# MaxLayar/Ray-Tracing-Extended

Hardware: AMD Instinct MI355X
Metric: Mrays/s (higher is better)
Workload: dtype f32; 1 GPU; configs[2]: Chess pieces x17 (100,440 triangles, BVH4), 1920x1080, 64 rays/pixel/frame (1024 spp = 16 frames), 8 bounces, PCG, FLAT_CHUNKS semantics; decomposition=single GPU, rays_per_frame=243378252, triangles=100440, chunks=7448, spheres=0

## Files before the change

ray-tracing-extended_amd/csrc/rt_api.hip:

```cpp
#include <hip/hip_runtime.h>

#include <algorithm>
#include <chrono>
#include <cfloat>
#include <cmath>
#include <condition_variable>
#include <deque>
#include <mutex>
#include <cstdarg>
#include <cstdio>
#include <cstring>
#include <ctime>
#include <string>
#include <thread>
#include <vector>

#include "rt_kernels.hpp"
#include "rt_stream.hpp"
namespace rtk {
const void* stream_kernel(bool counting, bool philox, bool compact, bool triangles);
const void* cam_stream_kernel(bool philox, bool compact, bool triangles);
}
#include "rt_geom.hpp"
#include "rt_bvh_gpu.hpp"
// ... 579 lines not shown
        return b ? lvl3(std::true_type{}) : lvl3(std::false_type{});
    };
    return a ? lvl2(std::true_type{}) : lvl2(std::false_type{});
}

struct LaunchPlan {
    rtk::DeviceScene S{}; rtk::FrameArgs F{}; rtk::StreamArgs A{};
    const void* fn = nullptr; size_t lds = 0;
    int grid = 1, batch = 1, ntiles = 0, sample_lanes_log2 = 0;
    bool philox = false, stream = false, tile_kernel = false, stream_sync = false, cam_table = false, record_costs = false;
};

int fill_scene(rt_ctx* c, rtk::DeviceScene& S)
{
    S.sph_geom = c->d_sph_geom.p; S.sph_mat = c->d_sph_mat.p; S.nodes = c->d_nodes.p; S.nodes_h = c->d_nodes_h.p;
    S.tri_geo = c->d_tri_geo.p; S.tri_nrm = c->d_tri_nrm.p; S.chunk_mat = c->d_chunk_mat.p; S.chunk_box = c->d_chunk_box.p;
    S.raw_tris = c->d_raw_tris.p; S.raw_chunk_range = c->d_raw_range.p;
    S.ns = (int)c->n_spheres; S.nn = (int)c->n_nodes;
    if (c->n_nodes >= ((size_t)1 << 25) || c->n_tris >= ((size_t)1 << 32) / 48)
        return fail(c, -7, "scene too large for 32-bit record offsets (%zu BVH nodes)", c->n_nodes);
    S.nt = (int)c->n_tris;
    S.nm = (int)c->n_chunks;
    return 0;
}

int tile_stack_cap(const rt_ctx* c)
{
    int cap = std::max(1, c->bvh.maxStack);
    if (c->opt_lds_stack > 0) cap = std::min(cap, c->opt_lds_stack);
    return std::min(cap, 64);
}

int plan_launch(rt_ctx* c, Variant var, int kernel, const rt_params* cams, int n_frames, LaunchPlan& P)
{
    rtk::DeviceScene& S = P.S; rtk::FrameArgs& F = P.F; rtk::StreamArgs& A = P.A;
    { int r = fill_scene(c, S); if (r) return r; }

    F.p = c->params;
    F.row0 = c->target_row0; F.nrows = c->target_rows; F.row_stride = c->target_row_stride;
    F.tile_w_log2 = 3;
    F.tiles_x = (c->target_w + 7) / 8; F.tiles_y = (c->target_rows + 7) / 8;
    if (kernel == 0 && c->opt_tile_w_log2 != 3) {
        F.tile_w_log2 = c->opt_tile_w_log2;
        const int tw = 1 << F.tile_w_log2, th = 64 >> F.tile_w_log2;
        F.tiles_x = (c->target_w + tw - 1) / tw; F.tiles_y = (c->target_rows + th - 1) / th;
    }
    const bool philox = P.philox = c->params.rngMode == RT_RNG_PHILOX && c->params.numRaysPerPixel >= 1;
    if (philox && var == Variant::Flat) return fail(c, -2, "the flat validation kernel implements the PCG stream only");
    if (philox) kernel = 1;
    if (philox && (c->target_w > 65535 || c->target_rows > 65535)) return fail(c, -7, "the Philox mode addresses at most 65535 x 65535 pixels per context");
    if (philox && (c->params.numRaysPerPixel > 65000 || c->params.maxBounceCount > 32000))
        return fail(c, -7, "the Philox mode takes at most 65000 rays per pixel per frame and 32000 bounces (sample and bounce share one signed 32-bit register)");
    const bool stream = P.stream = kernel == 1 && var != Variant::Flat && c->params.numRaysPerPixel >= 1
                                   && c->target_w <= 65535 && c->target_rows <= 65535;
    const bool tile_kernel = P.tile_kernel = !stream && var != Variant::Flat;
    F.stack_cap = tile_kernel ? tile_stack_cap(c)
                              : std::max(1, c->bvh.maxStack) + (stream ? 3 : 0);
    const bool six_waves = stream && !philox && var == Variant::Fast && c->opt_compact_nodes != 0 && c->n_nodes > 0;
    const int stream_stack = c->opt_stream_stack > 0 ? c->opt_stream_stack : (six_waves ? 24 : 30);
    const bool stream_spill = stream && F.stack_cap > stream_stack;
    if (stream_spill) F.stack_cap = stream_stack;
    F.full_sort = c->opt_full_sort;
    bool fixed_origin = camera_origin_is_fixed(c->params);
    if (cams) for (int f = 0; f < n_frames; ++f) fixed_origin = fixed_origin && camera_origin_is_fixed(cams[f]);
    F.fixed_origin = fixed_origin ? 1 : 0;
    F.out_frame = c->d_frame.p; F.accum = c->d_accum.p;
    F.tile_counter = c->d_tile_counter; F.counters = c->d_counters;

    const size_t lds = P.lds = var == Variant::Flat ? 0
                                       : (size_t)F.stack_cap * 64 * sizeof(uint32_t) * rtk::kWavesPerBlock
                                         + (stream ? (size_t)rtk::kGroupMax * sizeof(uint2) * rtk::kWavesPerBlock : 0);
    if (lds > 160 * 1024) return fail(c, -7, "BVH needs a %d-entry traversal stack: exceeds the 160 KiB LDS", F.stack_cap);
    const bool counting = var == Variant::Counting;
    const bool compact = c->opt_compact_nodes != 0;
    P.cam_table = cams != nullptr;
    const void* fn = P.fn = var == Variant::Flat ? (const void*)rtk::k_trace<false, true>
                   : stream ? (cams ? rtk::cam_stream_kernel(philox, compact, c->n_nodes > 0)
                                    : rtk::stream_kernel(counting, philox, compact, c->n_nodes > 0))
                   : c->n_nodes == 0
                            ? dispatch3(counting, false, false, [](auto C, auto, auto) { return (const void*)rtk::k_trace<decltype(C)::value, false, false, 6>; })
                            : dispatch3(counting, false, compact, [](auto C, auto, auto H) { return (const void*)rtk::k_trace<decltype(C)::value, false, decltype(H)::value>; });
    if (lds > 64 * 1024) RT_HIP(c, hipFuncSetAttribute(fn, hipFuncAttributeMaxDynamicSharedMemorySize, (int)lds));
    int per_cu = 0;
    RT_HIP(c, hipOccupancyMaxActiveBlocksPerMultiprocessor(&per_cu, fn, rtk::kBlock, lds));
    if (per_cu < 1) return fail(c, -7, "kernel does not fit a CU (LDS %zu B)", lds);
    P.ntiles = F.tiles_x * F.tiles_y;
    P.sample_lanes_log2 = !philox ? 0 : c->params.numRaysPerPixel >= 16 ? 4 : c->params.numRaysPerPixel >= 4 ? 2 : 0;
    const bool stream_sync = P.stream_sync = stream && (c->opt_tile_sync || philox);
    if (cams && !stream_sync) return fail(c, -7, "per-frame cameras: no k_cam_stream launch for this target");
    const size_t frames_in_queue = ((stream_sync && c->opt_frame_batch != 1) ? (size_t)std::max(1, std::min(n_frames, 64)) : 1) << P.sample_lanes_log2;
    const int want = (int)std::min<size_t>(((size_t)P.ntiles * frames_in_queue + rtk::kWavesPerBlock - 1) / rtk::kWavesPerBlock, (size_t)1 << 20);
    if (c->opt_blocks_per_cu > 0) per_cu = std::min(per_cu, c->opt_blocks_per_cu);
    const int grid = P.grid = std::max(1, std::min(want, per_cu * c->n_cu));
    A.shade_threshold = std::max(1, std::min(64, c->opt_shade_threshold));
    A.total_pixels = (unsigned int)P.ntiles * 64u;
    A.tile_sync = stream_sync ? 1 : 0;
    A.sample_lanes_log2 = P.sample_lanes_log2;
    A.tiles_per_fetch = std::max(1, std::min(rtk::kGroupMax, c->opt_tiles_per_fetch));
    A.guide_div = 1;
    A.node_min = std::max(1, std::min(64, c->opt_node_min));
    const unsigned int gstack_stride = (unsigned int)grid * rtk::kBlock;
    if (philox) {
        RT_HIP(c, c->d_park.ensure((size_t)grid * rtk::kWavesPerBlock * (size_t)A.tiles_per_fetch * 192));
        F.park = c->d_park.p;
    }
    if (stream_spill) {
        RT_HIP(c, c->d_gstack.ensure((size_t)(c->bvh.maxStack + 3 - F.stack_cap) * gstack_stride));
        F.gstack = c->d_gstack.p; F.gstack_stride = gstack_stride;
    }
    if (tile_kernel && c->bvh.maxStack > F.stack_cap) {
        RT_HIP(c, c->d_gstack.ensure((size_t)(c->bvh.maxStack - F.stack_cap) * gstack_stride));
        F.gstack = c->d_gstack.p; F.gstack_stride = gstack_stride;
// ... 1328 lines not shown
```

ray-tracing-extended_amd/csrc/rt_kernels.hpp:

```cpp
#pragma once
#include <cstddef>
#include <type_traits>
#include "rt_math.hpp"
#include "bvh.hpp"
#include "../../include/rt.h"

namespace rtk {

using rtm::v3;

struct DeviceScene {
    const float4* sph_geom;
    const float4* sph_mat;
    const float4* nodes;
    const float4* nodes_h;
    const float4* tri_geo;
    const float4* tri_nrm;
    const float4* chunk_mat;
    const float4* chunk_box;
    const float*  raw_tris;
    const uint32_t* raw_chunk_range;
    int ns, nn, nt, nm;
};

// ... 16 lines not shown
    float4* out_frame;
    float4* accum;
    float* park;
    const uint4* primary;
    const float4* focus;
    unsigned int* tile_counter;
    unsigned long long* counters;
};

constexpr uint32_t kNone = 0xFFFFFFFFu;
constexpr uint32_t kTriBit = 0x80000000u;

struct Hit {
    float    t;
    uint32_t id;
    float    u, v;
};

struct TravStack {
    uint32_t* lds; uint32_t* glb; int cap; unsigned int stride;
    __device__ __forceinline__ void push(int& sp, uint32_t v) const
    {
        if (sp < cap) lds[sp * 64] = v; else glb[(size_t)(sp - cap) * stride] = v;
        ++sp;
    }
    __device__ __forceinline__ uint32_t pop(int& sp) const
    {
        --sp;
        return sp < cap ? lds[sp * 64] : glb[(size_t)(sp - cap) * stride];
    }
};

__device__ __forceinline__ unsigned long long ballot_(bool pred) { return __builtin_amdgcn_ballot_w64(pred); }
__device__ __forceinline__ unsigned long long ballot2_(bool a, bool b) { return __builtin_amdgcn_ballot_w64(a) & __builtin_amdgcn_ballot_w64(b); }

#define RT_REGION_LIST(X) X(loop) X(fetch) X(shade) X(hit) X(hit_sphere) X(hit_checker) X(hit_scatter) X(env) X(env_sun) X(camera) X(pixel_done) \
                          X(take) X(refill) X(setup) X(setup_list) X(burst) X(burstiter) X(nodeloop) X(node) X(node_spill) X(node_pop) X(leaf) X(tri) \
                          X(tri_accept) X(tri_tie) X(tri_chunk) X(prologue) X(verify) X(epilogue) X(camera_dof) X(camera_focus) X(setup_spheres)
enum Region : int {
#define RT_X(NAME) R_##NAME,
    RT_REGION_LIST(RT_X)
#undef RT_X
    kRegionsUsed
};
constexpr int kNumRegions = 32;
static_assert(kRegionsUsed <= kNumRegions, "rt_stats.regionExecs holds 32 regions");
struct Counters { uint32_t rays, sph, nodes, tris, hits; uint32_t phase_lanes[5], phase_execs[5]; uint32_t region[kNumRegions]; };
constexpr int kNumCounters = 15 + kNumRegions;

#ifdef RT_MARKERS
#define RT_MARK(TEXT) asm volatile("; RTMARK " TEXT)
#define RT_RARE_PATH() asm volatile("; RTRARE")
#define RT_RARE_PATH_EXPR() ({ asm volatile("; RTRARE"); 0; })
#else
#define RT_MARK(TEXT) do { } while (0)
#define RT_RARE_PATH() do { } while (0)
#define RT_RARE_PATH_EXPR() 0
#endif
#define RT_REGION_BEGIN(NAME) do { RT_MARK("begin " #NAME); if (COUNT) { const unsigned long long rm_ = rtk::ballot_(true); \
                                   if ((unsigned)__builtin_ctzll(rm_) == (threadIdx.x & 63u)) cnt.region[rtk::R_##NAME]++; } } while (0)
#define RT_REGION_END(NAME) RT_MARK("end " #NAME)

template <bool COUNT>
__device__ __forceinline__ void phase_tick(Counters& cnt, int k)
{
    if (COUNT) {
        cnt.phase_lanes[k]++;
        const unsigned long long m = ballot_(1);
        if ((unsigned)(__builtin_ctzll(m)) == (threadIdx.x & 63u)) cnt.phase_execs[k]++;
    }
}

__device__ __forceinline__ v3 ld3(const float* p) { return rtm::mk(p[0], p[1], p[2]); }

__device__ __forceinline__ bool ray_bounding_box(v3 o, v3 inv, v3 bmin, v3 bmax)
{
    float tminx = (bmin.x - o.x) * inv.x, tminy = (bmin.y - o.y) * inv.y, tminz = (bmin.z - o.z) * inv.z;
    float tmaxx = (bmax.x - o.x) * inv.x, tmaxy = (bmax.y - o.y) * inv.y, tmaxz = (bmax.z - o.z) * inv.z;
    float t1x = rtm::fmin_(tminx, tmaxx), t1y = rtm::fmin_(tminy, tmaxy), t1z = rtm::fmin_(tminz, tmaxz);
    float t2x = rtm::fmax_(tminx, tmaxx), t2y = rtm::fmax_(tminy, tmaxy), t2z = rtm::fmax_(tminz, tmaxz);
    float tNear = rtm::fmax_(rtm::fmax_(t1x, t1y), t1z);
    float tFar  = rtm::fmin_(rtm::fmin_(t2x, t2y), t2z);
    return tNear <= tFar;
}

struct SphereA { float a, den, rden; bool den_ok; };
__device__ __forceinline__ SphereA sphere_a(float a)
{
    SphereA s; s.a = a; s.den = 2.0f * a;
    s.den_ok = s.den >= 0x1p-60f && s.den <= 0x1p60f;
    s.rden = rtm::rcp_mid(s.den);
    return s;
}
__device__ __forceinline__ bool ray_sphere(v3 o, v3 d, const SphereA& sa, v3 centre, float radius, float& dst)
{
    v3 oc = o - centre;
    float b = 2.0f * rtm::dot(oc, d);
    float c = rtm::dot(oc, oc) - radius * radius;
    float disc = b * b - 4.0f * sa.a * c;
    if (disc >= 0.0f) {
        const float num = -b - rtm::sqrt_(disc);
        const float an = __builtin_fabsf(num);
        const float q0 = num * sa.rden;
        float q = __builtin_fmaf(__builtin_fmaf(-q0, sa.den, num), sa.rden, q0);
        q = (num == 0.0f) ? q0 : q;
        if (!(sa.den_ok && (num == 0.0f || (an >= 0x1p-60f && an <= 0x1p60f)))) { RT_COLD_PATH(); q = num / sa.den; }
        dst = q;
        return dst >= 0.0f;
    }
    return false;
}

__device__ __forceinline__ bool ray_triangle(v3 o, v3 d, v3 A, v3 eAB, v3 eAC, v3 n, float& dst, float& u, float& v)
{
    v3 ao = o - A;
    v3 dao = rtm::cross(ao, d);
    float det = -rtm::dot(d, n);
    float inv = rtm::rcp_mid(det);
    if (det > 0x1p100f) { RT_COLD_PATH(); inv = 1.0f / det; }
    dst = rtm::dot(ao, n) * inv;
    u = rtm::dot(eAC, dao) * inv;
    v = -rtm::dot(eAB, dao) * inv;
    float w = 1.0f - u - v;
    return det >= 1e-6f && dst >= 0.0f && u >= 0.0f && v >= 0.0f && w >= 0.0f;
}


template <bool H> struct RaySlabT;
template <> struct RaySlabT<false> {
    v3 inv;
    v3 oinv;
    uint32_t nx, ny, nz;
    uint32_t fx, fy, fz;
};
template <> struct RaySlabT<true> {
    v3 inv, oinv;
    uint32_t nxy, fxy, zo;
};
using RaySlab = RaySlabT<false>;

template <bool H = false>
__device__ __forceinline__ RaySlabT<H> make_slab(v3 o, v3 d)
{
    RaySlabT<H> r;
    r.inv = rtm::mk(rtm::rcp_(d.x), rtm::rcp_(d.y), rtm::rcp_(d.z));
    r.oinv = rtm::mk(o.x * r.inv.x, o.y * r.inv.y, o.z * r.inv.z);
    if constexpr (H) {
        r.nxy = (d.x < 0.0f ? 16u : 0u) + (d.y < 0.0f ? 32u : 0u);
        r.fxy = 48u - r.nxy;
        r.zo = d.z < 0.0f ? 80u : 64u;
    } else {
        r.nx = d.x < 0.0f ? 48u : 0u;
        r.ny = d.y < 0.0f ? 64u : 16u;
        r.nz = d.z < 0.0f ? 80u : 32u;
        r.fx = 48u - r.nx; r.fy = 80u - r.ny; r.fz = 112u - r.nz;
    }
    return r;
}

typedef _Float16 rt_half2 __attribute__((ext_vector_type(2)));
__device__ __forceinline__ rt_half2 as_half2(uint32_t u) { return __builtin_bit_cast(rt_half2, u); }

template <bool H>
__device__ __forceinline__ void node_step(const float4* __restrict__ nodes, uint32_t cur, const RaySlabT<H>& r, float best_t, bool full_sort,
                                          float& t0, float& t1, float& t2, float& t3,
                                          uint32_t& c0, uint32_t& c1, uint32_t& c2, uint32_t& c3)
{
    const char* nb = reinterpret_cast<const char*>(nodes);
    const uint32_t base = cur << 7;
    const float INF = __builtin_inff();
    if constexpr (H) {
        const uint4 na = *reinterpret_cast<const uint4*>(nb + (base + r.nxy)), fa = *reinterpret_cast<const uint4*>(nb + (base + r.fxy));
        const uint4 zz = *reinterpret_cast<const uint4*>(nb + (base + r.zo));
        const uint4 ch = *reinterpret_cast<const uint4*>(nb + (base + 96u));
        const float4 og = *reinterpret_cast<const float4*>(nb + (base + 112u));
        c0 = ch.x; c1 = ch.y; c2 = ch.z; c3 = ch.w;
#ifdef RT_PROBE_LOADS
        for (int k_ = 0; k_ < RT_PROBE_LOADS; ++k_) (void)*reinterpret_cast<const volatile uint32_t*>(nb + (base + 124u));
#endif
#ifdef RT_PROBE_VALU
        { float pa_ = r.inv.x; for (int k_ = 0; k_ < RT_PROBE_VALU; ++k_) asm volatile("v_fma_f32 %0, %0, %0, %0" : "+v"(pa_)); }
#endif
#ifdef RT_PROBE_VALU_HALF
        { float pa_ = r.inv.x; for (int k_ = 0; k_ < RT_PROBE_VALU_HALF; ++k_) asm volatile("v_max_f32 %0, %0, %0" : "+v"(pa_)); }
#endif
        const float kx = __builtin_fmaf(og.x, r.inv.x, -r.oinv.x), ky = __builtin_fmaf(og.y, r.inv.y, -r.oinv.y), kz = __builtin_fmaf(og.z, r.inv.z, -r.oinv.z);
#define RT_SLABH(XW, YW, ZNW, ZFW, E, TK)                                                                                 \
        {                                                                                                                \
            const float nx_ = __builtin_fmaf((float)as_half2(na.XW).E, r.inv.x, kx), fx_ = __builtin_fmaf((float)as_half2(fa.XW).E, r.inv.x, kx); \
            const float ny_ = __builtin_fmaf((float)as_half2(na.YW).E, r.inv.y, ky), fy_ = __builtin_fmaf((float)as_half2(fa.YW).E, r.inv.y, ky); \
            const float nz_ = __builtin_fmaf((float)as_half2(zz.ZNW).E, r.inv.z, kz), fz_ = __builtin_fmaf((float)as_half2(zz.ZFW).E, r.inv.z, kz); \
            const float tn_ = __builtin_fmaxf(__builtin_fmaxf(__builtin_fmaxf(nx_, ny_), nz_), 0.0f);                    \
            const float tf_ = __builtin_fminf(__builtin_fminf(__builtin_fminf(fx_, fy_), fz_), best_t);                  \
            TK = (tn_ <= tf_) ? tn_ : INF;                                                                               \
        }
        RT_SLABH(x, z, x, z, x, t0) RT_SLABH(x, z, x, z, y, t1) RT_SLABH(y, w, y, w, x, t2) RT_SLABH(y, w, y, w, y, t3)
#undef RT_SLABH
    } else {
    const float4 px = *reinterpret_cast<const float4*>(nb + (base + r.nx)), qx = *reinterpret_cast<const float4*>(nb + (base + r.fx));
    const float4 py = *reinterpret_cast<const float4*>(nb + (base + r.ny)), qy = *reinterpret_cast<const float4*>(nb + (base + r.fy));
    const float4 pz = *reinterpret_cast<const float4*>(nb + (base + r.nz)), qz = *reinterpret_cast<const float4*>(nb + (base + r.fz));
    const uint4 ch = *reinterpret_cast<const uint4*>(nb + (base + 96u));
    c0 = ch.x; c1 = ch.y; c2 = ch.z; c3 = ch.w;
#ifdef RT_PROBE_LOADS
    for (int k_ = 0; k_ < RT_PROBE_LOADS; ++k_) (void)*reinterpret_cast<const volatile uint32_t*>(nb + (base + 124u));
#endif
#ifdef RT_PROBE_VALU
    { float pa_ = r.inv.x; for (int k_ = 0; k_ < RT_PROBE_VALU; ++k_) asm volatile("v_fma_f32 %0, %0, %0, %0" : "+v"(pa_)); }
#endif
#define RT_SLAB(K, TK)                                                                                                   \
    {                                                                                                                    \
        const float nx_ = __builtin_fmaf(px.K, r.inv.x, -r.oinv.x), fx_ = __builtin_fmaf(qx.K, r.inv.x, -r.oinv.x);      \
        const float ny_ = __builtin_fmaf(py.K, r.inv.y, -r.oinv.y), fy_ = __builtin_fmaf(qy.K, r.inv.y, -r.oinv.y);      \
        const float nz_ = __builtin_fmaf(pz.K, r.inv.z, -r.oinv.z), fz_ = __builtin_fmaf(qz.K, r.inv.z, -r.oinv.z);      \
        const float tn_ = __builtin_fmaxf(__builtin_fmaxf(__builtin_fmaxf(nx_, ny_), nz_), 0.0f);                        \
        const float tf_ = __builtin_fminf(__builtin_fminf(__builtin_fminf(fx_, fy_), fz_), best_t);                      \
        TK = (tn_ <= tf_) ? tn_ : INF;                                                                                   \
    }
    RT_SLAB(x, t0) RT_SLAB(y, t1) RT_SLAB(z, t2) RT_SLAB(w, t3)
#undef RT_SLAB
    }
#define RT_CSWAP(TA, CA, TB, CB) { const bool s_ = TB < TA; const float tt_ = s_ ? TB : TA, tu_ = s_ ? TA : TB;         \
                                   const uint32_t ct_ = s_ ? CB : CA, cu_ = s_ ? CA : CB; TA = tt_; TB = tu_; CA = ct_; CB = cu_; }
    RT_CSWAP(t0, c0, t1, c1) RT_CSWAP(t2, c2, t3, c3) RT_CSWAP(t0, c0, t2, c2)
    if (full_sort) { RT_RARE_PATH(); RT_CSWAP(t1, c1, t3, c3) RT_CSWAP(t1, c1, t2, c2) }
#undef RT_CSWAP
// ... 391 lines not shown
```

ray-tracing-extended_amd/csrc/rt_stream.hpp:

```cpp
#pragma once
#include "rt_kernels.hpp"

namespace rtk {

struct StreamArgs {
    int shade_threshold;
    unsigned int total_pixels;
    int node_min;
    int tiles_per_fetch;
    int guide_div;
    int tile_sync;
    int n16, n4, n1;
    int sample_lanes_log2;
};

enum : uint32_t { kModeTrav = 0, kModeShade = 1, kModeDead = 2, kModeWait = 3, kModeTravStrict = 0xFFFFFFFFu };
__device__ __forceinline__ bool is_trav(uint32_t mode) { return (int)mode <= 0; }
constexpr uint32_t kNoPixel = 0xFFFFFFFFu;

struct StreamKernArgs { DeviceScene S; FrameArgs F; StreamArgs A; };
static_assert(alignof(StreamArgs) <= 8, "kernarg layout = struct layout");
static_assert(offsetof(StreamKernArgs, F) == ((sizeof(DeviceScene) + 7) & ~size_t(7))
              && offsetof(StreamKernArgs, A) == ((offsetof(StreamKernArgs, F) + sizeof(FrameArgs) + 7) & ~size_t(7)), "kernarg layout = struct layout");

struct CamRecord {
    float4 view;
    float4 m0, m1, m2;
    float4 pos;
};
struct StreamCamKernArgs { DeviceScene S; FrameArgs F; StreamArgs A; const CamRecord* cams; };
static_assert(offsetof(StreamCamKernArgs, A) == offsetof(StreamKernArgs, A)
              && offsetof(StreamCamKernArgs, cams) == ((offsetof(StreamCamKernArgs, A) + sizeof(StreamArgs) + 7) & ~size_t(7)), "kernarg layout = struct layout");

#ifndef RT_STREAM_WAVES
#define RT_STREAM_WAVES 6
#endif
#ifndef RT_STREAM_WAVES_PHILOX
#define RT_STREAM_WAVES_PHILOX 5
#endif
constexpr int stream_waves(bool count, bool philox, bool h, bool tri) { return count ? 3 : !tri ? 6 : philox ? RT_STREAM_WAVES_PHILOX : !h ? 5 : RT_STREAM_WAVES; }


template <bool COUNT, bool PHILOX = false, bool H = false, bool TRI = true>
__global__ __launch_bounds__(kBlock) __attribute__((amdgpu_waves_per_eu(stream_waves(COUNT, PHILOX, H, TRI), stream_waves(COUNT, PHILOX, H, TRI)))) void k_stream(DeviceScene S, FrameArgs F, StreamArgs A)
{
    constexpr bool CAMS = false;
#include "rt_stream_body.hpp"
}

template <bool PHILOX, bool H, bool TRI>
__global__ __launch_bounds__(kBlock) __attribute__((amdgpu_waves_per_eu(stream_waves(false, PHILOX, H, TRI), stream_waves(false, PHILOX, H, TRI)))) void k_cam_stream(DeviceScene S, FrameArgs F, StreamArgs A, const CamRecord* cams)
{
    constexpr bool COUNT = false, CAMS = true;
    (void)cams;
#include "rt_stream_body.hpp"
}

}
```

ray-tracing-extended_amd/csrc/rt_stream_body.hpp:

```cpp
    extern __shared__ uint32_t lds_stack[];
    RT_MARK("begin prologue");
    const int lane = threadIdx.x & 63, wave = threadIdx.x >> 6;
    uint32_t* stk = lds_stack + (size_t)wave * F.stack_cap * 64 + lane;
    const int cap = F.stack_cap;
    uint32_t* const gstk = F.gstack ? F.gstack + (blockIdx.x * kBlock + threadIdx.x) : nullptr;
    using lds_u32 = __attribute__((address_space(3))) uint32_t;
    const uint32_t stk0 = (uint32_t)(uintptr_t)(lds_u32*)stk;
    uint32_t top = stk0;
    auto slot = [](uint32_t a) -> lds_u32& { return *reinterpret_cast<lds_u32*>((uintptr_t)a); };
    const uint32_t capb = (uint32_t)cap << 8;
    auto pop = [&]() -> uint32_t {
        top -= 256u;
        if (gstk == nullptr) return slot(top);
        RT_RARE_PATH();
        const uint32_t depth = top - stk0;
        uint32_t v = slot(stk0 + min(depth, capb - 256u));
        asm volatile("" : "+v"(v));
        if (depth >= capb) { RT_RARE_PATH(); v = gstk[(size_t)((depth - capb) >> 8) * F.gstack_stride]; }
        return v;
    };
    typedef uint32_t u32x2 __attribute__((ext_vector_type(2)));
    using lds_u2 = __attribute__((address_space(3))) u32x2;
    lds_u2* const item_tab = reinterpret_cast<lds_u2*>((uintptr_t)__builtin_amdgcn_readfirstlane(
                                 (uint32_t)(uintptr_t)(lds_u32*)(lds_stack + (size_t)kWavesPerBlock * F.stack_cap * 64) + (uint32_t)wave * (kGroupMax * 8u)));
    Counters cnt = {};
    const float INF = __builtin_inff();
    auto park_slot = [&](const FrameArgs& F, const StreamArgs& A, unsigned int k) -> float* {
        return F.park + (((size_t)(blockIdx.x * kWavesPerBlock) + (threadIdx.x >> 6)) * (unsigned)A.tiles_per_fetch + k) * 192u;
    };

    uint32_t mode = A.tile_sync ? kModeWait : kModeShade;
    bool fresh = false;
    uint32_t pxy = kNoPixel;
    uint32_t rng = 0u;
    int sample = 0, bounce = 0;
    v3 total = rtm::mk(0.f, 0.f, 0.f), light = total, rayColour = total, o = total, d = total;
    RaySlabT<H> slab = make_slab<H>(rtm::mk(0.f, 0.f, 0.f), rtm::mk(1.f, 1.f, 1.f));
    uint32_t cur = kNone;
    Hit best; best.t = INF; best.id = kNone; best.u = 0.f; best.v = 0.f;
    bool live = false;
    unsigned long long wave_t0 = 0;
    unsigned int group_base = 0, group_len = 0;
    unsigned int next_unit = 0;
    unsigned int kidx = 0;

    auto decode = [](const FrameArgs& F, const StreamArgs& A, unsigned int item, unsigned int& tile, unsigned int& sub, unsigned int& frame0) -> int {
        const unsigned int ntiles_ = (unsigned)(F.tiles_x * F.tiles_y);
        if constexpr (PHILOX) {
            const int sgl = A.sample_lanes_log2;
            const unsigned int per_frame = ntiles_ << sgl;
            const unsigned int g = item / per_frame, r = item - g * per_frame;
            tile = r >> sgl; sub = r & ((1u << sgl) - 1u); frame0 = g;
            return sgl;
        }
        const unsigned int items1_ = (unsigned)A.n1 * ntiles_, items4_ = (unsigned)A.n4 * (ntiles_ << 2);
        int fgl = 0; unsigned int fbase = (unsigned)A.n16 * 16u + (unsigned)A.n4 * 4u;
        if (item >= items1_) { item -= items1_; fgl = 2; fbase = (unsigned)A.n16 * 16u; if (item >= items4_) { item -= items4_; fgl = 4; fbase = 0u; } }
        const unsigned int per_group = ntiles_ << fgl;
        const unsigned int g = item / per_group, r = item - g * per_group;
        tile = r >> fgl; sub = r & ((1u << fgl) - 1u); frame0 = fbase + (g << fgl);
        return fgl;
    };
    auto pixel_index = [&](const FrameArgs& F) -> uint32_t {
        const int ly = (int)(pxy >> 16);
        return (uint32_t)(F.row0 + (ly >> 3) * F.row_stride + (ly & 7)) * (uint32_t)F.p.width + (pxy & 0xFFFFu);
    };
    auto start_pixel = [&](const FrameArgs& F, const StreamArgs& A, unsigned int id) -> bool {
        const rt_params& p = F.p;
        const uint32_t W = (uint32_t)p.width;
        const unsigned int nframes_ = (unsigned)(A.n16 * 16 + A.n4 * 4 + A.n1);
        const u32x2 e = item_tab[id >> 6];
        const unsigned int pos = id & 63u;
        const int fgl = (int)(e.y >> 28);
        const unsigned int frame0 = e.y & 0x0FFFFFFFu;
        const int pxl = 6 - fgl, swl = pxl >> 1;
        const unsigned int pix = pos & ((1u << pxl) - 1u);
        const unsigned int fi = PHILOX ? frame0 : frame0 + (pos >> pxl);
        const int x = (int)((e.x & 0xFFFFu) + (pix & ((1u << swl) - 1u)));
        const int yy = (int)((e.x >> 16) + (pix >> swl));
        if (!(x < p.width && yy < F.nrows && fi < nframes_)) return false;
        pxy = (uint32_t)x | ((uint32_t)yy << 16); kidx = id | (fi << 16);
        const uint32_t pixelIndex = (uint32_t)(F.row0 + (yy >> 3) * F.row_stride + (yy & 7)) * W + (uint32_t)x;
        if constexpr (PHILOX) sample = (int)(pos >> pxl);
        else { rng = pixelIndex + (uint32_t)(F.frame + (int)fi) * 719393u; sample = 0; }
        total = rtm::mk(0.f, 0.f, 0.f);
        live = false;
        return true;
    };
// ... 104 lines not shown
            RT_REGION_BEGIN(shade);
            const StreamKernArgs& KA = fresh_kernargs<StreamKernArgs>();
            const DeviceScene& S = KA.S; const FrameArgs& F = KA.F; const StreamArgs& A = KA.A;
            const rt_params& p = F.p;
            const float* M = p.camLocalToWorld;
            const uint32_t W = (uint32_t)p.width;
            bool need_ray = false;
            bool want = false;
            bool retrace = false;
            if (mode == kModeShade) {
                need_ray = fresh;
                fresh = false;
                bool path_done = false;
                if constexpr (TRI) {
                    if (live && best.id != kNone && (best.id & kTriBit) && p.intersectMode == RT_INTERSECT_FLAT_CHUNKS) {
                        RT_REGION_BEGIN(verify);
                        const uint32_t chunk = __float_as_uint(S.tri_nrm[(size_t)(best.id & ~kTriBit) * 3].w);
                        const float4 bmn = S.chunk_box[(size_t)chunk * 2], bmx = S.chunk_box[(size_t)chunk * 2 + 1];
                        if (!ray_bounding_box(o, slab.inv, rtm::mk(bmn.x, bmn.y, bmn.z), rtm::mk(bmx.x, bmx.y, bmx.z))) { retrace = true; live = false; }
                        RT_REGION_END(verify);
                    }
                }
                if (live) {
                    if (best.id != kNone) {
                        RT_REGION_BEGIN(hit);
                        phase_tick<COUNT>(cnt, 2);
                        if (COUNT) cnt.hits++;
                        const v3 hitPoint = o + d * best.t;
                        v3 normal; const float4* mat;
                        if (best.id & kTriBit) {
                            const uint32_t ti = best.id & ~kTriBit;
                            const float4* tn = S.tri_nrm + (size_t)ti * 3;
                            const float4 n0 = tn[0], n1 = tn[1], n2 = tn[2];
                            const float w = 1.0f - best.u - best.v;
                            normal = rtm::normalize((rtm::mk(n0.x, n0.y, n0.z) * w + rtm::mk(n1.x, n1.y, n1.z) * best.u)
                                                    + rtm::mk(n2.x, n2.y, n2.z) * best.v);
                            mat = S.chunk_mat + (size_t)__float_as_uint(n0.w) * 4;
                        } else {
                            RT_REGION_BEGIN(hit_sphere);
                            const float4 s = S.sph_geom[best.id];
                            normal = rtm::normalize(hitPoint - rtm::mk(s.x, s.y, s.z));
                            mat = S.sph_mat + (size_t)best.id * 4;
                            RT_REGION_END(hit_sphere);
                        }
                        const float4 mcol = mat[0], memi = mat[1], mprm = mat[3];
                        const int flag = (int)__float_as_uint(mprm.w);
                        v3 colour = rtm::mk(mcol.x, mcol.y, mcol.z);
                        bool skip = false;
                        if (flag == 1) {
                            RT_REGION_BEGIN(hit_checker);
                            float cx = mod2(__builtin_floorf(hitPoint.x)), cz = mod2(__builtin_floorf(hitPoint.z));
                            if (!(cx == cz)) colour = rtm::mk(memi.x, memi.y, memi.z);
                            RT_REGION_END(hit_checker);
                        } else if (flag == 2 && (PHILOX ? (sample >> 16) : bounce) == 0) {
                            o = hitPoint + d * 0.001f;
                            skip = true;
                        }
                        if (!skip) {
                            RT_REGION_BEGIN(hit_scatter);
                            auto scatter = [&](auto& R) {
                                const bool isSpecular = mprm.z >= rtm::random_value(R);
                                const float specF = isSpecular ? 1.0f : 0.0f;
                                o = hitPoint;
                                v3 diffuseDir = rtm::normalize(normal + rtm::random_direction(R));
                                const float4 mspec = mat[2];
                                v3 specularDir = rtm::reflect(d, normal);
                                d = rtm::normalize(rtm::lerp(diffuseDir, specularDir, mprm.y * specF));
                                v3 emitted = rtm::mk(memi.x, memi.y, memi.z) * mprm.x;
                                light = light + emitted * rayColour;
                                rayColour = rayColour * rtm::lerp(colour, rtm::mk(mspec.x, mspec.y, mspec.z), specF);
                                float pr = rtm::fmax_(rayColour.x, rtm::fmax_(rayColour.y, rayColour.z));
                                if (rtm::random_value(R) >= pr) path_done = true;
                                else { float ip = rtm::rcp_(pr); rayColour = rayColour * ip; }
                            };
                            if constexpr (PHILOX) {
                                rtm::PhiloxScope R;
                                R.begin(pixel_index(F), (uint32_t)F.frame + (kidx >> 16), (uint32_t)sample & 0xFFFFu, 1u + 2u * ((uint32_t)sample >> 16));
                                scatter(R);
                            } else scatter(rng);
                            RT_REGION_END(hit_scatter);
                        }
                        if constexpr (PHILOX) { sample += 0x10000; if ((sample >> 16) > p.maxBounceCount) path_done = true; }
                        else { ++bounce; if (bounce > p.maxBounceCount) path_done = true; }
                        RT_REGION_END(hit);
                    } else {
                        RT_REGION_BEGIN(env);
#if !defined(RT_DIAG_IDLE) && !defined(RT_DIAG_PRIMARY) && !defined(RT_DIAG_TOP)
                        phase_tick<COUNT>(cnt, 3);
#endif
                        light = light + environment_light(p, d) * rayColour;
                        path_done = true;
                        RT_REGION_END(env);
                    }
                    if (path_done) {
                        total = total + light;
                        if constexpr (PHILOX) sample = (sample & 0xFFFF) + (1 << A.sample_lanes_log2); else ++sample;
                        if (PHILOX && sample >= p.numRaysPerPixel) {
                            float* q = park_slot(F, A, (kidx & 0xFFFFu) >> 6) + (kidx & 63u);
                            q[0] = total.x; q[64] = total.y; q[128] = total.z;
                            pxy = kNoPixel; want = true;
                        } else if (sample >= p.numRaysPerPixel) {
                            RT_REGION_BEGIN(pixel_done);
                            const float n = (float)p.numRaysPerPixel;
                            const float cx = total.x / n, cy = total.y / n, cz = total.z / n;
                            const size_t pi = (size_t)(pxy >> 16) * W + (pxy & 0xFFFFu);
                            float one = 1.0f;
                            asm volatile("" : "+v"(one));
                            F.out_frame[(size_t)(kidx >> 16) * F.frame_stride + pi] = make_float4(cx, cy, cz, one);
                            if (F.frames_in_launch <= 1) {
                                const float weight = 1.0f / (float)(F.frame + 1);
                                const float omw = 1.0f - weight;
                                const float4 prev = F.accum[pi];
                                float4 acc;
                                acc.x = rtm::saturate(prev.x * omw + cx * weight);
                                acc.y = rtm::saturate(prev.y * omw + cy * weight);
                                acc.z = rtm::saturate(prev.z * omw + cz * weight);
                                acc.w = rtm::saturate(prev.w * omw + 1.0f * weight);
                                F.accum[pi] = acc;
                            }
                            pxy = kNoPixel; want = A.tile_sync != 0;
                            RT_REGION_END(pixel_done);
                        } else need_ray = true;
                    }
                    live = false;
                }
            }
            if (ballot_(want) != 0ull) {
                RT_REGION_BEGIN(take);
                const bool got = take_units(F, A, want);
                if (want) { if (got) need_ray = true; else mode = kModeWait; }
                RT_REGION_END(take);
            }
            if (mode == kModeShade) {
                while (!PHILOX && !A.tile_sync) {
                    const unsigned long long need = ballot_(pxy == kNoPixel && mode != kModeDead);
                    if (need == 0) break;
                    RT_REGION_BEGIN(refill);
                    if (pxy == kNoPixel && mode != kModeDead) {
                        unsigned int base = 0;
                        const int first = __builtin_ctzll(need);
                        if (lane == first) base = atomicAdd(F.tile_counter, (unsigned int)__popcll(need));
                        base = __shfl(base, first, 64);
                        const unsigned int idx = base + (unsigned int)__popcll(need & ((1ull << lane) - 1ull));
                        if (idx >= A.total_pixels) mode = kModeDead;
                        else {
                            const unsigned int tile = idx >> 6, within = idx & 63u;
                            const int x = (int)(tile % (unsigned)F.tiles_x) * 8 + (int)(within & 7u);
                            const int yy = (int)(tile / (unsigned)F.tiles_x) * 8 + (int)(within >> 3);
                            if (x < p.width && yy < F.nrows) {
                                pxy = (uint32_t)x | ((uint32_t)yy << 16);
                                const int y = F.row0 + (yy >> 3) * F.row_stride + (yy & 7);
                                rng = ((uint32_t)y * W + (uint32_t)x) + (uint32_t)F.frame * 719393u;
                                total = rtm::mk(0.f, 0.f, 0.f);
                                sample = 0;
                                need_ray = true;
                            }
                        }
                    }
                    RT_REGION_END(refill);
                }
                if (mode == kModeShade) {
                    if (need_ray) {
                        RT_REGION_BEGIN(camera);
#if !defined(RT_DIAG_IDLE) && !defined(RT_DIAG_PRIMARY) && !defined(RT_DIAG_TOP)
                        phase_tick<COUNT>(cnt, 4);
#endif
                        Camera cam;
                        cam.W = (float)W;
                        if constexpr (CAMS) {
                        auto rec = [&]() { return fresh_kernargs<StreamCamKernArgs>().cams + (kidx >> 16); };
                        const int px = (int)(pxy & 0xFFFFu), ly = (int)(pxy >> 16);
                        const int y = F.row0 + (ly >> 3) * F.row_stride + (ly & 7);
                        const float4 vw = rec()->view;
                        const float uvx = ((float)px + 0.5f) / cam.W, uvy = ((float)y + 0.5f) / (float)(uint32_t)p.height;
                        const float lx = (uvx - 0.5f) * vw.x, lyv = (uvy - 0.5f) * vw.y, lz = 1.0f * vw.z;
                        const float4 r0 = rec()->m0;
                        const float fx = ((r0.x * lx + r0.y * lyv) + r0.z * lz) + r0.w * 1.0f;
                        const float4 r1 = rec()->m1;
                        const float fy = ((r1.x * lx + r1.y * lyv) + r1.z * lz) + r1.w * 1.0f;
                        const float4 r2 = rec()->m2;
                        cam.focusPoint = rtm::mk(fx, fy, ((r2.x * lx + r2.y * lyv) + r2.z * lz) + r2.w * 1.0f);
                        const CamRecord* rc = rec();
                        cam.right = rtm::mk(rc->m0.x, rc->m1.x, rc->m2.x);
                        cam.up    = rtm::mk(rc->m0.y, rc->m1.y, rc->m2.y);
                        const float4 pv = rc->pos;
                        cam.pos   = rtm::mk(pv.x, pv.y, pv.z);
                        if constexpr (PHILOX) {
                            rtm::PhiloxScope R;
                            R.begin((uint32_t)y * W + (uint32_t)px, (uint32_t)F.frame + (kidx >> 16), (uint32_t)sample & 0xFFFFu, 0u);
                            camera_ray(p, cam, R, o, d, F.fixed_origin != 0);
                        } else camera_ray(p, cam, rng, o, d, F.fixed_origin != 0);
                        } else {
                        cam.right = rtm::mk(M[0], M[4], M[8]);
                        cam.up    = rtm::mk(M[1], M[5], M[9]);
                        cam.pos   = ld3(p.worldSpaceCameraPos);
                        const int px = (int)(pxy & 0xFFFFu), ly = (int)(pxy >> 16);
                        const int y = F.row0 + (ly >> 3) * F.row_stride + (ly & 7);
#ifdef RT_AB_NO_FOCUS
                        if (false) {
#else
                        if (F.focus != nullptr) {
#endif
                            const float4 fpt = F.focus[(size_t)ly * W + (uint32_t)px];
                            cam.focusPoint = rtm::mk(fpt.x, fpt.y, fpt.z);
                        } else {
                        RT_MARK("begin camera_focus");
                        const float uvx = ((float)px + 0.5f) / cam.W, uvy = ((float)y + 0.5f) / (float)(uint32_t)p.height;
                        const float lx = (uvx - 0.5f) * p.viewParams[0], lyv = (uvy - 0.5f) * p.viewParams[1], lz = 1.0f * p.viewParams[2];
                        cam.focusPoint = rtm::mk(((M[0] * lx + M[1] * lyv) + M[2]  * lz) + M[3]  * 1.0f,
                                                 ((M[4] * lx + M[5] * lyv) + M[6]  * lz) + M[7]  * 1.0f,
                                                 ((M[8] * lx + M[9] * lyv) + M[10] * lz) + M[11] * 1.0f);
                        RT_MARK("end camera_focus");
                        }
                        if constexpr (PHILOX) {
                            rtm::PhiloxScope R;
                            R.begin((uint32_t)y * W + (uint32_t)px, (uint32_t)F.frame + (kidx >> 16), (uint32_t)sample & 0xFFFFu, 0u);
                            camera_ray(p, cam, R, o, d, F.fixed_origin != 0);
                        } else camera_ray(p, cam, rng, o, d, F.fixed_origin != 0);
                        }
                        if constexpr (PHILOX) sample &= 0xFFFF; else bounce = 0;
                        rayColour = rtm::mk(1.f, 1.f, 1.f); light = rtm::mk(0.f, 0.f, 0.f);
                        RT_REGION_END(camera);
                    }
                    {
                        RT_REGION_BEGIN(setup);
                        if (!retrace) cnt.rays++;
                        best.t = INF; best.id = kNone;
                        const float a = rtm::dot(d, d);
                        const SphereA sa = sphere_a(a);
                        for (int i = 0; i < S.ns; ++i) {
                            RT_REGION_BEGIN(setup_spheres);
                            const float4 s = S.sph_geom[i];
                            float dst;
                            if (COUNT && !retrace) cnt.sph++;
                            if (ray_sphere(o, d, sa, rtm::mk(s.x, s.y, s.z), s.w, dst) && dst < best.t) { best.t = dst; best.id = (uint32_t)i; }
                            RT_REGION_END(setup_spheres);
                        }
                        live = true;
                        const bool traceable = ray_traceable(o, d, a);
                        if constexpr (TRI) {
                            if (S.nn > 0 && traceable) {
                                slab = make_slab<H>(o, d);
                                cur = 0; top = stk0; mode = retrace ? kModeTravStrict : kModeTrav;
                                if (F.primary != nullptr && need_ray) {
                                    RT_REGION_BEGIN(setup_list);
                                    const uint4 L = F.primary[(size_t)(pxy >> 16) * W + (pxy & 0xFFFFu)];
                                    if (L.x != 0xFFFFFFFEu) {
                                        cur = L.x;
                                        slot(top) = L.w; top = (L.w != kNone) ? top + 256u : top;
                                        slot(top) = L.z; top = (L.z != kNone) ? top + 256u : top;
                                        slot(top) = L.y; top = (L.y != kNone) ? top + 256u : top;
                                        if (L.x == kNone) mode = kModeShade;
                                    }
                                    RT_REGION_END(setup_list);
                                }
                            }
                        }
                        RT_REGION_END(setup);
                    }
                }
            }
            RT_REGION_END(shade);
        } else {
            if constexpr (TRI) {
            __builtin_amdgcn_s_setprio(1);
            RT_REGION_BEGIN(burst);
            for (;;) {
                RT_REGION_BEGIN(burstiter);
                for (;;) {
                    RT_REGION_BEGIN(nodeloop);
                    const int nAtNode = __popcll(ballot_((int)cur >= 0));
                    if (nAtNode == 0) { RT_REGION_END(nodeloop); break; }
                    if (nAtNode < A.node_min && ballot2_(is_trav(mode), (int)cur < 0) != 0) { RT_REGION_END(nodeloop); break; }
#ifdef RT_DIAG_IDLE
                    if (COUNT) {
                        if (is_trav(mode) && (int)cur < 0) cnt.phase_lanes[3]++;
                        if (mode == kModeShade) cnt.phase_lanes[4]++;
                        if (lane == 0) { cnt.phase_execs[3]++; cnt.phase_execs[4]++; }
                    }
#endif
                    if ((int)cur >= 0) {
                        RT_REGION_BEGIN(node);
                        if (COUNT) cnt.nodes++;
                        phase_tick<COUNT>(cnt, 0);
#ifdef RT_DIAG_TOP
                        if (COUNT && cur < (uint32_t)RT_DIAG_TOP) { cnt.phase_lanes[3]++; }
                        if (COUNT && cur < 4u * RT_DIAG_TOP + 1u) { cnt.phase_lanes[4]++; }
                        if (COUNT && ballot_(cur >= (uint32_t)RT_DIAG_TOP) == 0ull && (unsigned)__builtin_ctzll(ballot_(true)) == (unsigned)lane) cnt.phase_execs[3]++;
                        if (COUNT && ballot_(cur >= 4u * RT_DIAG_TOP + 1u) == 0ull && (unsigned)__builtin_ctzll(ballot_(true)) == (unsigned)lane) cnt.phase_execs[4]++;
#endif
#ifdef RT_DIAG_PRIMARY
                        if (COUNT && (PHILOX ? (sample >> 16) : bounce) == 0) { cnt.phase_lanes[3]++; if ((unsigned)__builtin_ctzll(ballot_(true)) == (unsigned)lane) cnt.phase_execs[3]++; }
#endif
                        float t0, t1, t2, t3;
                        uint32_t c0, c1, c2, c3;
                        node_step<H>(H ? S.nodes_h : S.nodes, cur, slab, best.t, F.full_sort != 0, t0, t1, t2, t3, c0, c1, c2, c3);
                        if (gstk == nullptr || ((void)RT_RARE_PATH_EXPR(), ballot_(top - stk0 + 768u > capb) == 0)) {
                            slot(top) = c3; top = (t3 < INF) ? top + 256u : top;
                            slot(top) = c2; top = (t2 < INF) ? top + 256u : top;
                            slot(top) = c1; top = (t1 < INF) ? top + 256u : top;
                        } else {
                            RT_REGION_BEGIN(node_spill);
                            auto push = [&](uint32_t c) {
                                const uint32_t depth = top - stk0;
                                if (depth < capb) slot(top) = c; else gstk[(size_t)((depth - capb) >> 8) * F.gstack_stride] = c;
                                top += 256u;
                            };
                            if (t3 < INF) push(c3);
                            if (t2 < INF) push(c2);
                            if (t1 < INF) push(c1);
                            RT_REGION_END(node_spill);
                        }
                        if (t0 < INF) cur = c0;
                        else {
                            RT_REGION_BEGIN(node_pop);
                            if (top != stk0) cur = pop();
                            else { cur = kNone; mode = kModeShade; }
                            RT_REGION_END(node_pop);
                        }
                        RT_REGION_END(node);
                    }
                    RT_REGION_END(nodeloop);
                }
                if (is_trav(mode) && (int)cur < 0) {
                    RT_REGION_BEGIN(leaf);
                    uint32_t ti = (cur & 0x7FFFFFFFu) >> 2;
                    const uint32_t last = ti + (cur & 3u);
                    if (cur != kNone)
                    for (; ti <= last; ++ti) {
                        RT_REGION_BEGIN(tri);
                        float4 g0, g1, g2;
                        load_tri(S.tri_geo, ti, g0, g1, g2);
                        float dst, u, v;
                        if (COUNT) cnt.tris++;
                        phase_tick<COUNT>(cnt, 1);
#ifdef RT_DIAG_PRIMARY
                        if (COUNT && (PHILOX ? (sample >> 16) : bounce) == 0) { cnt.phase_lanes[4]++; if ((unsigned)__builtin_ctzll(ballot_(true)) == (unsigned)lane) cnt.phase_execs[4]++; }
#endif
                        const bool hit = ray_triangle(o, d, rtm::mk(g0.x, g0.y, g0.z), rtm::mk(g0.w, g1.x, g1.y),
                                                      rtm::mk(g1.z, g1.w, g2.x), rtm::mk(g2.y, g2.z, g2.w), dst, u, v);
                        if (hit && dst <= best.t) {
                            RT_REGION_BEGIN(tri_accept);
                            bool take = dst < best.t;
                            if (!take && (best.id & kTriBit) && best.id != kNone) {
                                RT_REGION_BEGIN(tri_tie);
                                uint32_t oc = __float_as_uint(S.tri_nrm[(size_t)ti * 3 + 1].w);
                                uint32_t ob = __float_as_uint(S.tri_nrm[(size_t)(best.id & ~kTriBit) * 3 + 1].w);
                                take = oc < ob;
                                RT_REGION_END(tri_tie);
                            }
                            if (take && mode == kModeTravStrict) {
                                RT_RARE_PATH();
                                RT_REGION_BEGIN(tri_chunk);
                                uint32_t chunk = __float_as_uint(S.tri_nrm[(size_t)ti * 3].w);
                                float4 bmn = S.chunk_box[(size_t)chunk * 2], bmx = S.chunk_box[(size_t)chunk * 2 + 1];
                                take = ray_bounding_box(o, slab.inv, rtm::mk(bmn.x, bmn.y, bmn.z), rtm::mk(bmx.x, bmx.y, bmx.z));
                                RT_REGION_END(tri_chunk);
                            }
                            if (take) { best.t = dst; best.id = kTriBit | ti; best.u = u; best.v = v; }
                            RT_REGION_END(tri_accept);
                        }
                        RT_REGION_END(tri);
                    }
                    if (top != stk0) cur = pop();
                    else { cur = kNone; mode = kModeShade; }
                    RT_REGION_END(leaf);
                }
                RT_REGION_END(burstiter);
                if (ballot_(is_trav(mode)) == 0) break;
                if ((int)__popcll(ballot_(mode == kModeShade)) >= thr) break;
            }
            RT_REGION_END(burst);
            }
        }
    }
    RT_MARK("begin epilogue");
    {
        unsigned long long v[kNumCounters] = { cnt.rays, cnt.sph, cnt.nodes, cnt.tris, cnt.hits };
        for (int k = 0; k < 5; ++k) { v[5 + k] = cnt.phase_lanes[k]; v[10 + k] = cnt.phase_execs[k]; }
        for (int k = 0; k < kNumRegions; ++k) v[15 + k] = cnt.region[k];
        for (int k = 0; k < (COUNT ? kNumCounters : 1); ++k) {
            unsigned long long s = v[k];
            for (int off = 32; off > 0; off >>= 1) s += __shfl_down(s, off, 64);
            if (lane == 0) atomicAdd(&fresh_kernargs<StreamKernArgs>().F.counters[k], s);
        }
    }
    RT_MARK("end epilogue");
```

Baseline: 20120 Mrays/s.

## Raise stream kernel to seven waves with smaller LDS stack and fewer registers

Raises the default stream wave count from six to seven per SIMD and shrinks the LDS traversal stack to 21 entries so the extra wave fits. It saves registers by packing the hierarchical slab offsets into one word and by folding the bounce counter into the upper half of the sample register, as the Philox path already did. It also adds a conservative per-wave stack-depth upper bound, so the spill check ballot runs only when the stack may be near capacity. In exchange, the smaller stack spills to global memory more often on deep traversals, and the bound logic adds some bookkeeping per node step.

```diff
diff --git a/ray-tracing-extended_amd/csrc/rt_api.hip b/ray-tracing-extended_amd/csrc/rt_api.hip
--- a/ray-tracing-extended_amd/csrc/rt_api.hip
+++ b/ray-tracing-extended_amd/csrc/rt_api.hip
@@ -655,12 +655,13 @@
     if (philox && (c->params.numRaysPerPixel > 65000 || c->params.maxBounceCount > 32000))
         return fail(c, -7, "the Philox mode takes at most 65000 rays per pixel per frame and 32000 bounces (sample and bounce share one signed 32-bit register)");
     const bool stream = P.stream = kernel == 1 && var != Variant::Flat && c->params.numRaysPerPixel >= 1
-                                   && c->target_w <= 65535 && c->target_rows <= 65535;
+                                   && c->target_w <= 65535 && c->target_rows <= 65535
+                                   && c->params.numRaysPerPixel <= 65000 && c->params.maxBounceCount <= 32000;
     const bool tile_kernel = P.tile_kernel = !stream && var != Variant::Flat;
     F.stack_cap = tile_kernel ? tile_stack_cap(c)
                               : std::max(1, c->bvh.maxStack) + (stream ? 3 : 0);
-    const bool six_waves = stream && !philox && var == Variant::Fast && c->opt_compact_nodes != 0 && c->n_nodes > 0;
-    const int stream_stack = c->opt_stream_stack > 0 ? c->opt_stream_stack : (six_waves ? 24 : 30);
+    const bool seven_waves = stream && !philox && var == Variant::Fast && c->opt_compact_nodes != 0 && c->n_nodes > 0;
+    const int stream_stack = c->opt_stream_stack > 0 ? c->opt_stream_stack : (seven_waves ? (RT_STREAM_WAVES >= 7 ? 21 : 24) : 30);
     const bool stream_spill = stream && F.stack_cap > stream_stack;
     if (stream_spill) F.stack_cap = stream_stack;
     F.full_sort = c->opt_full_sort;
diff --git a/ray-tracing-extended_amd/csrc/rt_kernels.hpp b/ray-tracing-extended_amd/csrc/rt_kernels.hpp
--- a/ray-tracing-extended_amd/csrc/rt_kernels.hpp
+++ b/ray-tracing-extended_amd/csrc/rt_kernels.hpp
@@ -92,10 +92,12 @@
 #define RT_MARK(TEXT) asm volatile("; RTMARK " TEXT)
 #define RT_RARE_PATH() asm volatile("; RTRARE")
 #define RT_RARE_PATH_EXPR() ({ asm volatile("; RTRARE"); 0; })
+#define RT_QUARTER_PATH() asm volatile("; RTQUARTER")
 #else
 #define RT_MARK(TEXT) do { } while (0)
 #define RT_RARE_PATH() do { } while (0)
 #define RT_RARE_PATH_EXPR() 0
+#define RT_QUARTER_PATH() do { } while (0)
 #endif
 #define RT_REGION_BEGIN(NAME) do { RT_MARK("begin " #NAME); if (COUNT) { const unsigned long long rm_ = rtk::ballot_(true); \
                                    if ((unsigned)__builtin_ctzll(rm_) == (threadIdx.x & 63u)) cnt.region[rtk::R_##NAME]++; } } while (0)
@@ -175,7 +177,7 @@
 };
 template <> struct RaySlabT<true> {
     v3 inv, oinv;
-    uint32_t nxy, fxy, zo;
+    uint32_t sets;
 };
 using RaySlab = RaySlabT<false>;
 
@@ -186,9 +188,7 @@
     r.inv = rtm::mk(rtm::rcp_(d.x), rtm::rcp_(d.y), rtm::rcp_(d.z));
     r.oinv = rtm::mk(o.x * r.inv.x, o.y * r.inv.y, o.z * r.inv.z);
     if constexpr (H) {
-        r.nxy = (d.x < 0.0f ? 16u : 0u) + (d.y < 0.0f ? 32u : 0u);
-        r.fxy = 48u - r.nxy;
-        r.zo = d.z < 0.0f ? 80u : 64u;
+        r.sets = ((d.x < 0.0f ? 16u : 0u) + (d.y < 0.0f ? 32u : 0u)) | (d.z < 0.0f ? 80u << 8 : 64u << 8);
     } else {
         r.nx = d.x < 0.0f ? 48u : 0u;
         r.ny = d.y < 0.0f ? 64u : 16u;
@@ -210,8 +210,9 @@
     const uint32_t base = cur << 7;
     const float INF = __builtin_inff();
     if constexpr (H) {
-        const uint4 na = *reinterpret_cast<const uint4*>(nb + (base + r.nxy)), fa = *reinterpret_cast<const uint4*>(nb + (base + r.fxy));
-        const uint4 zz = *reinterpret_cast<const uint4*>(nb + (base + r.zo));
+        const uint32_t nxy = r.sets & 0xFFu;
+        const uint4 na = *reinterpret_cast<const uint4*>(nb + (base + nxy)), fa = *reinterpret_cast<const uint4*>(nb + (base + (nxy ^ 48u)));
+        const uint4 zz = *reinterpret_cast<const uint4*>(nb + (base + (r.sets >> 8)));
         const uint4 ch = *reinterpret_cast<const uint4*>(nb + (base + 96u));
         const float4 og = *reinterpret_cast<const float4*>(nb + (base + 112u));
         c0 = ch.x; c1 = ch.y; c2 = ch.z; c3 = ch.w;
diff --git a/ray-tracing-extended_amd/csrc/rt_stream.hpp b/ray-tracing-extended_amd/csrc/rt_stream.hpp
--- a/ray-tracing-extended_amd/csrc/rt_stream.hpp
+++ b/ray-tracing-extended_amd/csrc/rt_stream.hpp
@@ -33,7 +33,7 @@
               && offsetof(StreamCamKernArgs, cams) == ((offsetof(StreamCamKernArgs, A) + sizeof(StreamArgs) + 7) & ~size_t(7)), "kernarg layout = struct layout");
 
 #ifndef RT_STREAM_WAVES
-#define RT_STREAM_WAVES 6
+#define RT_STREAM_WAVES 7
 #endif
 #ifndef RT_STREAM_WAVES_PHILOX
 #define RT_STREAM_WAVES_PHILOX 5
diff --git a/ray-tracing-extended_amd/csrc/rt_stream_body.hpp b/ray-tracing-extended_amd/csrc/rt_stream_body.hpp
--- a/ray-tracing-extended_amd/csrc/rt_stream_body.hpp
+++ b/ray-tracing-extended_amd/csrc/rt_stream_body.hpp
@@ -9,9 +9,10 @@
     uint32_t top = stk0;
     auto slot = [](uint32_t a) -> lds_u32& { return *reinterpret_cast<lds_u32*>((uintptr_t)a); };
     const uint32_t capb = (uint32_t)cap << 8;
+    uint32_t ub = 0u;
     auto pop = [&]() -> uint32_t {
         top -= 256u;
-        if (gstk == nullptr) return slot(top);
+        if (gstk == nullptr || ub <= capb) return slot(top);
         RT_RARE_PATH();
         const uint32_t depth = top - stk0;
         uint32_t v = slot(stk0 + min(depth, capb - 256u));
@@ -33,7 +34,7 @@
     bool fresh = false;
     uint32_t pxy = kNoPixel;
     uint32_t rng = 0u;
-    int sample = 0, bounce = 0;
+    int sample = 0;
     v3 total = rtm::mk(0.f, 0.f, 0.f), light = total, rayColour = total, o = total, d = total;
     RaySlabT<H> slab = make_slab<H>(rtm::mk(0.f, 0.f, 0.f), rtm::mk(1.f, 1.f, 1.f));
     uint32_t cur = kNone;
@@ -244,7 +245,7 @@
                             float cx = mod2(__builtin_floorf(hitPoint.x)), cz = mod2(__builtin_floorf(hitPoint.z));
                             if (!(cx == cz)) colour = rtm::mk(memi.x, memi.y, memi.z);
                             RT_REGION_END(hit_checker);
-                        } else if (flag == 2 && (PHILOX ? (sample >> 16) : bounce) == 0) {
+                        } else if (flag == 2 && (sample >> 16) == 0) {
                             o = hitPoint + d * 0.001f;
                             skip = true;
                         }
@@ -272,12 +273,12 @@
                             } else scatter(rng);
                             RT_REGION_END(hit_scatter);
                         }
-                        if constexpr (PHILOX) { sample += 0x10000; if ((sample >> 16) > p.maxBounceCount) path_done = true; }
-                        else { ++bounce; if (bounce > p.maxBounceCount) path_done = true; }
+                        sample += 0x10000;
+                        if ((sample >> 16) > p.maxBounceCount) path_done = true;
                         RT_REGION_END(hit);
                     } else {
                         RT_REGION_BEGIN(env);
-#if !defined(RT_DIAG_IDLE) && !defined(RT_DIAG_PRIMARY) && !defined(RT_DIAG_TOP)
+#if !defined(RT_DIAG_IDLE) && !defined(RT_DIAG_PRIMARY) && !defined(RT_DIAG_TOP) && !defined(RT_DIAG_STACK)
                         phase_tick<COUNT>(cnt, 3);
 #endif
                         light = light + environment_light(p, d) * rayColour;
@@ -286,7 +287,7 @@
                     }
                     if (path_done) {
                         total = total + light;
-                        if constexpr (PHILOX) sample = (sample & 0xFFFF) + (1 << A.sample_lanes_log2); else ++sample;
+                        sample = (sample & 0xFFFF) + (PHILOX ? 1 << A.sample_lanes_log2 : 1);
                         if (PHILOX && sample >= p.numRaysPerPixel) {
                             float* q = park_slot(F, A, (kidx & 0xFFFFu) >> 6) + (kidx & 63u);
                             q[0] = total.x; q[64] = total.y; q[128] = total.z;
@@ -354,7 +355,7 @@
                 if (mode == kModeShade) {
                     if (need_ray) {
                         RT_REGION_BEGIN(camera);
-#if !defined(RT_DIAG_IDLE) && !defined(RT_DIAG_PRIMARY) && !defined(RT_DIAG_TOP)
+#if !defined(RT_DIAG_IDLE) && !defined(RT_DIAG_PRIMARY) && !defined(RT_DIAG_TOP) && !defined(RT_DIAG_STACK)
                         phase_tick<COUNT>(cnt, 4);
 #endif
                         Camera cam;
@@ -410,7 +411,7 @@
                             camera_ray(p, cam, R, o, d, F.fixed_origin != 0);
                         } else camera_ray(p, cam, rng, o, d, F.fixed_origin != 0);
                         }
-                        if constexpr (PHILOX) sample &= 0xFFFF; else bounce = 0;
+                        sample &= 0xFFFF;
                         rayColour = rtm::mk(1.f, 1.f, 1.f); light = rtm::mk(0.f, 0.f, 0.f);
                         RT_REGION_END(camera);
                     }
@@ -452,6 +453,7 @@
                     }
                 }
             }
+            ub = max(ub, 768u);
             RT_REGION_END(shade);
         } else {
             if constexpr (TRI) {
@@ -471,6 +473,21 @@
                         if (lane == 0) { cnt.phase_execs[3]++; cnt.phase_execs[4]++; }
                     }
 #endif
+                    bool plain = true;
+                    if (gstk != nullptr) {
+                        if (ub + 768u > capb) {
+                            RT_QUARTER_PATH();
+                            const uint32_t depth = top - stk0, low = capb > 2304u ? capb - 2304u : 0u;
+#ifdef RT_DIAG_STACK
+                            if (COUNT) { const bool above_ = ballot_(depth > low) != 0; if (lane == 0) { cnt.phase_execs[3]++; if (above_) cnt.phase_lanes[4]++; } }
+#endif
+                            if (ballot_(depth > low) == 0) ub = low;
+                            else if (ballot_(depth + 768u > capb) == 0) ub = capb - 768u;
+                            else ub = min(ub, 0x40000000u);
+                        }
+                        plain = ub + 768u <= capb;
+                        ub += 768u;
+                    }
                     if ((int)cur >= 0) {
                         RT_REGION_BEGIN(node);
                         if (COUNT) cnt.nodes++;
@@ -482,16 +499,20 @@
                         if (COUNT && ballot_(cur >= 4u * RT_DIAG_TOP + 1u) == 0ull && (unsigned)__builtin_ctzll(ballot_(true)) == (unsigned)lane) cnt.phase_execs[4]++;
 #endif
 #ifdef RT_DIAG_PRIMARY
-                        if (COUNT && (PHILOX ? (sample >> 16) : bounce) == 0) { cnt.phase_lanes[3]++; if ((unsigned)__builtin_ctzll(ballot_(true)) == (unsigned)lane) cnt.phase_execs[3]++; }
+                        if (COUNT && (sample >> 16) == 0) { cnt.phase_lanes[3]++; if ((unsigned)__builtin_ctzll(ballot_(true)) == (unsigned)lane) cnt.phase_execs[3]++; }
 #endif
                         float t0, t1, t2, t3;
                         uint32_t c0, c1, c2, c3;
                         node_step<H>(H ? S.nodes_h : S.nodes, cur, slab, best.t, F.full_sort != 0, t0, t1, t2, t3, c0, c1, c2, c3);
-                        if (gstk == nullptr || ((void)RT_RARE_PATH_EXPR(), ballot_(top - stk0 + 768u > capb) == 0)) {
+#ifdef RT_DIAG_STACK
+                        if (COUNT && gstk != nullptr && ballot_(top - stk0 + 768u > capb) != 0 && (unsigned)__builtin_ctzll(ballot_(true)) == (unsigned)lane) cnt.phase_execs[4]++;
+#endif
+                        if (plain) {
                             slot(top) = c3; top = (t3 < INF) ? top + 256u : top;
                             slot(top) = c2; top = (t2 < INF) ? top + 256u : top;
                             slot(top) = c1; top = (t1 < INF) ? top + 256u : top;
                         } else {
+                            RT_RARE_PATH();
                             RT_REGION_BEGIN(node_spill);
                             auto push = [&](uint32_t c) {
                                 const uint32_t depth = top - stk0;
@@ -503,6 +524,11 @@
                             if (t1 < INF) push(c1);
                             RT_REGION_END(node_spill);
                         }
+#ifdef RT_DIAG_STACK
+                        if (COUNT) {
+                            cnt.phase_lanes[3] = max(cnt.phase_lanes[3], (top - stk0) >> 8);
+                        }
+#endif
                         if (t0 < INF) cur = c0;
                         else {
                             RT_REGION_BEGIN(node_pop);
@@ -527,7 +553,7 @@
                         if (COUNT) cnt.tris++;
                         phase_tick<COUNT>(cnt, 1);
 #ifdef RT_DIAG_PRIMARY
-                        if (COUNT && (PHILOX ? (sample >> 16) : bounce) == 0) { cnt.phase_lanes[4]++; if ((unsigned)__builtin_ctzll(ballot_(true)) == (unsigned)lane) cnt.phase_execs[4]++; }
+                        if (COUNT && (sample >> 16) == 0) { cnt.phase_lanes[4]++; if ((unsigned)__builtin_ctzll(ballot_(true)) == (unsigned)lane) cnt.phase_execs[4]++; }
 #endif
                         const bool hit = ray_triangle(o, d, rtm::mk(g0.x, g0.y, g0.z), rtm::mk(g0.w, g1.x, g1.y),
                                                       rtm::mk(g1.z, g1.w, g2.x), rtm::mk(g2.y, g2.z, g2.w), dst, u, v);
@@ -573,6 +599,13 @@
         for (int k = 0; k < kNumRegions; ++k) v[15 + k] = cnt.region[k];
         for (int k = 0; k < (COUNT ? kNumCounters : 1); ++k) {
             unsigned long long s = v[k];
+#ifdef RT_DIAG_STACK
+            if (k == 8) {
+                for (int off = 32; off > 0; off >>= 1) s = max(s, (unsigned long long)__shfl_down(s, off, 64));
+                if (lane == 0) atomicMax(&fresh_kernargs<StreamKernArgs>().F.counters[k], s);
+                continue;
+            }
+#endif
             for (int off = 32; off > 0; off >>= 1) s += __shfl_down(s, off, 64);
             if (lane == 0) atomicAdd(&fresh_kernargs<StreamKernArgs>().F.counters[k], s);
         }
```

Measured after the change: 21200 Mrays/s, median of 6. 5.3% higher.
